# MiraPurkrabek/ProbPose_code

Hardware: AMD Instinct MI355X
Metric: person-crops/sec @ 256x192 bs64 (higher is better)
Workload: dtype f16x3; 1 GPU; ProbPose-small (ViT-S 12x384, 12 heads x 32) bs64 random 256x192 uint8 crops per GPU, flip_test=True, seeded random-init weights: preprocess -> backbone x2 passes -> ProbMapHead (heatmap branch + Sparsemax + 4 towers) -> ProbMap decode -> results in pinned host memory; crops_per_gpu=64, global_batch=64, parallelism=dp1, steps_in_flight=2

## Files before the change

probpose_code_amd/csrc/pp_panel_split.hip:

```cpp
#include "pp_common.h"
#include "pp_device.h"
#include "pp_gemm.h"
#include "pp_split.h"

#include <cstdlib>

namespace pp {
namespace psplit {

#ifndef PSPLIT_DBG
#define PSPLIT_DBG 0
#endif
constexpr int DBG = PSPLIT_DBG;

constexpr int THREADS = 512;
constexpr int CST_BYTES = 48 * 1024;
constexpr int lds_bytes(int BM, int BN, int NST) { return NST * (BM + BN) * 128 + (NST == 2 ? CST_BYTES : 0); }
template <bool SPLIT>
__device__ __forceinline__ f32x4 mma(const u32x4& a, const u32x4& b, f32x4 c) {
    return SPLIT ? mma_f16(a, b, c) : mma_bf16(a, b, c);
}

template <int GATHER, int RF, int CF, bool SPLIT, int NST, bool HEAD = false, bool POOL = false>
__global__ __launch_bounds__(THREADS, 2) void panel_split_kernel(const GemmParams p) {
    constexpr int ESZ = SPLIT ? 4 : 2;
    constexpr int KS = 128 / ESZ;
    constexpr int BM = 32 * RF, BN = 64 * CF;
    constexpr int NA = BM / 8, JA = NA / 8;
    constexpr int STAGE = (BM + BN) * 128;
    constexpr int NI = (BM + BN) / 64;
    constexpr int OFF_CST = NST * STAGE;
    static_assert(NST == 2 || NST == 3, "two or three stages");
    static_assert((BM / 4) * BN * 4 <= (NST == 2 ? CST_BYTES : STAGE), "a quarter of the fp32 tile fits the staging region");
    static_assert(lds_bytes(BM, BN, NST) <= 160 * 1024, "LDS");
    static_assert(NA % 8 == 0 && JA <= 4 && RF % 2 == 0 && (BM + BN) % 64 == 0, "instruction split");
    extern __shared__ __attribute__((aligned(16))) char smem[];
    const int tid = threadIdx.x, lane = tid & 63;
    const int wv = __builtin_amdgcn_readfirstlane(tid >> 6);
    const int rg = wv >> 2, cg = wv & 3;
    const int f_row = lane & 15, f_kg = lane >> 4;

    const int ntn = p.N / BN, ntm = (p.M + BM - 1) / BM;
    const int ntiles = ntn * ntm * p.groups;
    const int nsteps = p.K / KS;
    const int cps = p.Cin / KS;
    const int nprob = p.ksplit > 1 ? p.groups / p.ksplit : p.groups;
    const int cslice = p.ksplit > 1 ? p.Cin / p.ksplit : p.Cin;

    auto decode_tile = [&](int t, int& z, int& m0, int& n0) __attribute__((always_inline)) {
        if ((ntiles & 7) == 0) t = (t & 7) * (ntiles >> 3) + (t >> 3);
        if (p.tile_order == 1) {
            m0 = (t % ntm) * BM;
            const int r = t / ntm;
            n0 = (r % ntn) * BN;
            z = r / ntn;
            return;
        }
        n0 = (t % ntn) * BN;
        const int r = t / ntn;
        z = r % p.groups;
        m0 = (r / p.groups) * BM;
    };

    const int d_l = lane >> 3;
    const unsigned d_kbytes = (unsigned)(((lane & 7) ^ d_l) << 4);
    unsigned a_voff[JA];
    int a_y[JA], a_x[JA];
    unsigned w_voff;
    __amdgpu_buffer_rsrc_t a_rsrc, w_rsrc;
    int i_tile = blockIdx.x, i_step = 0, i_tap = 0, i_c0 = 0, i_py = 0, i_px = 0, i_cbeg = 0;
    bool i_live = true;
    auto setup_issue_tile = [&]() __attribute__((always_inline)) {
        int z = 0, m0 = 0, n0 = 0;
        i_live = i_tile < ntiles;
        if (i_live) decode_tile(i_tile, z, m0, n0);
        i_cbeg = 0;
        if (p.ksplit > 1) {
            i_cbeg = (z / nprob) * cslice;
            z = z % nprob;
        }
        if (GATHER == G_DECONV) {
            i_py = p.py < 0 ? (z >> 1) : p.py;
            i_px = p.py < 0 ? (z & 1) : p.px;
        }
        const char* Act = reinterpret_cast<const char*>(p.A) + (size_t)z * p.strideA_z * ESZ;
        const char* Wt = reinterpret_cast<const char*>(p.W) + (size_t)z * p.strideW_z * ESZ;
        a_rsrc = buffer_rsrc(Act, p.a_bytes);
        w_rsrc = buffer_rsrc(Wt, p.w_bytes);
#pragma unroll
        for (int j = 0; j < JA; ++j) {
            const int m = m0 + 8 * (wv + 8 * j) + d_l;
            const bool ok = i_live && m < p.M;
            if (GATHER == G_LINEAR) {
                a_y[j] = ok ? 0 : -100000;
                a_x[j] = 0;
                a_voff[j] = (unsigned)m * (unsigned)(p.lda * ESZ) + d_kbytes;
            } else {
                const int hw = p.H * p.Wd;
                const int b = m / hw, rr = m - b * hw;
                a_y[j] = ok ? rr / p.Wd : -100000;
                a_x[j] = rr - (rr / p.Wd) * p.Wd;
                a_voff[j] = (unsigned)m * (unsigned)(p.Cin * ESZ) + d_kbytes;
            }
        }
        w_voff = (unsigned)(n0 + 8 * (wv + 8 * JA - NA) + d_l) * (unsigned)(p.ldw * ESZ) + d_kbytes;
        i_step = 0;
        i_tap = 0;
        i_c0 = i_cbeg;
    };
    auto issue_instr = [&](int buf, int j) __attribute__((always_inline)) {
        char* dst = smem + buf * STAGE + (wv + 8 * j) * 1024;
        if (j < JA) {
            int dy = 0, dx = 0;
            if (GATHER == G_CONV3) {
                dy = i_tap / 3 - 1;
                dx = i_tap - (i_tap / 3) * 3 - 1;
            } else if (GATHER == G_DECONV) {
                dy = (i_tap >> 1) - 1 + i_py;
                dx = (i_tap & 1) - 1 + i_px;
            }
            const int jj = j < JA ? j : 0;
            const int yy = a_y[jj] + dy, xx = a_x[jj] + dx;
            const bool ok = GATHER == G_LINEAR ? a_y[jj] >= 0 : (yy >= 0 && yy < p.H && xx >= 0 && xx < p.Wd);
            const int tap_off = GATHER == G_LINEAR ? i_c0 * ESZ : ((dy * p.Wd + dx) * p.Cin + i_c0) * ESZ;
            const unsigned va = ok ? (unsigned)((int)a_voff[jj] + tap_off) : kOob;
            dma16(a_rsrc, dst, va);
        } else {
            const unsigned kb = (unsigned)((i_tap * p.Cin + i_c0) * ESZ) + (unsigned)((j - JA) * 64) * (unsigned)(p.ldw * ESZ);
            dma16(w_rsrc, dst, i_live ? w_voff + kb : kOob);
        }
    };
    const int ntaps = p.K / cslice;
    auto advance_cursor = [&]() __attribute__((always_inline)) {
        const bool ti = p.tap_inner != 0;
        const int tap = i_tap + (ti ? 1 : 0), c0 = i_c0 + (ti ? 0 : KS);
        const bool wrap = ti ? tap == ntaps : c0 == i_cbeg + cslice;
        i_tap = ti ? (wrap ? 0 : tap) : tap + (wrap ? 1 : 0);
        i_c0 = ti ? c0 + (wrap ? KS : 0) : (wrap ? i_cbeg : c0);
        if (++i_step == nsteps) {
            i_tile += gridDim.x;
            setup_issue_tile();
        }
    };
    (void)cps;

    const int sw = f_row & 7;
    const int a_frag_off = (rg * (BM / 2) + f_row) * 128;
    const int w_frag_off = BM * 128 + (cg * (BN / 4) + f_row) * 128;
    auto frag_a = [&](int buf, int lo, int rf) __attribute__((always_inline)) -> u32x4 {
        return *reinterpret_cast<const u32x4*>(smem + buf * STAGE + (((lo * 4 + f_kg) ^ sw) << 4) + a_frag_off + rf * 2048);
    };
    auto frag_w = [&](int buf, int lo, int cf) __attribute__((always_inline)) -> u32x4 {
        return *reinterpret_cast<const u32x4*>(smem + buf * STAGE + (((lo * 4 + f_kg) ^ sw) << 4) + w_frag_off + cf * 2048);
    };

    if ((int)blockIdx.x >= ntiles) return;

    constexpr int HP_PITCH = 100, HP_MAXN = 28;
    constexpr int OFF_HEADB = 4 * HP_MAXN * HP_PITCH * 4;
    static_assert(!HEAD || (SPLIT && GATHER == G_DECONV && RF == 6 && CF == 4 && NST == 2 && OFF_HEADB + 128 <= CST_BYTES), "fused 1x1 head");
    u32x4 hw[HEAD ? 2 : 1][2][2];
    if constexpr (HEAD) {
#pragma unroll
        for (int kb2 = 0; kb2 < 2; ++kb2)
#pragma unroll
            for (int nf = 0; nf < 2; ++nf)
#pragma unroll
                for (int hl = 0; hl < 2; ++hl)
                    hw[kb2][nf][hl] = *reinterpret_cast<const u32x4*>(reinterpret_cast<const char*>(p.head_w) +
                                                                      ((size_t)(((cg * 2 + kb2) * 2 + nf) * 2 + hl) * 64 + lane) * 16);
        if (tid < HP_MAXN) reinterpret_cast<float*>(smem + OFF_CST + OFF_HEADB)[tid] = tid < p.head_n ? p.head_b[tid] : 0.f;
    }
    setup_issue_tile();
#pragma unroll
    for (int s = 0; s < NST; ++s) {
#pragma unroll
        for (int j = 0; j < NI; ++j) issue_instr(s, j);
        advance_cursor();
    }
    wait_vm_lgkm<(NST - 1) * NI>();
    __builtin_amdgcn_s_barrier();
    int cb = 0;
    u32x4 ah[RF], wh[CF], al[RF], wl[CF];
#pragma unroll
    for (int cf = 0; cf < CF; ++cf) wh[cf] = frag_w(0, 0, cf);
#pragma unroll
    for (int rf = 0; rf < RF; ++rf) ah[rf] = frag_a(0, 0, rf);

    for (int tile = blockIdx.x; tile < ntiles; tile += gridDim.x) {
        f32x4 acc[CF][RF];
#pragma unroll
        for (int cf = 0; cf < CF; ++cf)
#pragma unroll
            for (int rf = 0; rf < RF; ++rf) acc[cf][rf] = f32x4{0.f, 0.f, 0.f, 0.f};
        f32x4 bias_r[CF];
        {
            int zb, mb, nb0;
            decode_tile(tile, zb, mb, nb0);
#pragma unroll
            for (int cf = 0; cf < CF; ++cf)
                bias_r[cf] = (p.bias && !(DBG & 1)) ? *reinterpret_cast<const f32x4*>(p.bias + (size_t)zb * p.strideBias_z + nb0 + cg * (BN / 4) + cf * 16 + f_kg * 4)
                                                    : f32x4{0.f, 0.f, 0.f, 0.f};
        }

        for (int k = 0; k < nsteps; ++k) {
            const int nb = cb + 1 == NST ? 0 : cb + 1;
            __builtin_amdgcn_sched_barrier(0);
#pragma unroll
            for (int cf = 0; cf < CF; ++cf) wl[cf] = frag_w(cb, 1, cf);
#pragma unroll
            for (int rf = 0; rf < RF; ++rf) al[rf] = frag_a(cb, 1, rf);
#pragma unroll
            for (int rf = 0; rf < RF; ++rf)
#pragma unroll
                for (int cf = 0; cf < CF; ++cf) acc[cf][rf] = mma<SPLIT>(wh[cf], ah[rf], acc[cf][rf]);
            __builtin_amdgcn_sched_barrier(0);
            wait_vm_lgkm<NST == 2 ? 0 : NI>();
            __builtin_amdgcn_s_barrier();
            __builtin_amdgcn_sched_barrier(0);
            if (NST == 2 || k + 1 < nsteps) {
#pragma unroll
                for (int j = 0; j < NI; ++j) issue_instr(cb, j);
                advance_cursor();
            }
            if constexpr (SPLIT) {
#pragma unroll
                for (int rf = 0; rf < RF; ++rf) {
#pragma unroll
                    for (int cf = 0; cf < CF; ++cf) acc[cf][rf] = mma<SPLIT>(wl[cf], ah[rf], acc[cf][rf]);
                    ah[rf] = frag_a(nb, 0, rf);
                }
#pragma unroll
                for (int cf = 0; cf < CF; ++cf) {
#pragma unroll
                    for (int rf = 0; rf < RF; ++rf) acc[cf][rf] = mma<SPLIT>(wh[cf], al[rf], acc[cf][rf]);
                    wh[cf] = frag_w(nb, 0, cf);
                }
            } else {
#pragma unroll
                for (int cf = 0; cf < CF; ++cf) wh[cf] = frag_w(nb, 0, cf);
#pragma unroll
                for (int rf = 0; rf < RF; ++rf) ah[rf] = frag_a(nb, 0, rf);
#pragma unroll
                for (int rf = 0; rf < RF; ++rf)
#pragma unroll
                    for (int cf = 0; cf < CF; ++cf) acc[cf][rf] = mma<SPLIT>(wl[cf], al[rf], acc[cf][rf]);
            }
            cb = nb;
        }
        const int last_buf = cb == 0 ? NST - 1 : cb - 1;

        if (DBG & 128) {
            f32x4 sum = acc[0][0];
#pragma unroll
            for (int cf = 0; cf < CF; ++cf)
#pragma unroll
                for (int rf = 0; rf < RF; ++rf) sum += acc[cf][rf];
            if (p.M < 0) reinterpret_cast<f32x4*>(p.C)[tid] = sum;
            if (NST == 3) {
#pragma unroll
                for (int j = 0; j < NI; ++j) issue_instr(last_buf, j);
                advance_cursor();
            }
            continue;
        }
        int lane_e = lane;
        asm volatile("" : "+v"(lane_e));
        const int e_row = lane_e & 15, e_kg = lane_e >> 4, tid_e = (tid & ~63) | lane_e;
        int z, m0, n0;
        decode_tile(tile, z, m0, n0);
        if constexpr (HEAD) {
            float* part = reinterpret_cast<float*>(smem + OFF_CST);
            const float* hb = reinterpret_cast<const float*>(smem + OFF_CST + OFF_HEADB);
            const int hwp = p.H * p.Wd;
            const int phase = p.py < 0 ? z : 2 * p.py + p.px;
#pragma unroll
            for (int r = 0; r < 2; ++r) {
                if (rg == r) {
#pragma unroll
                    for (int rf = 0; rf < RF; ++rf) {
                        f32x4 o0 = {0.f, 0.f, 0.f, 0.f}, o1 = {0.f, 0.f, 0.f, 0.f};
#pragma unroll
                        for (int kb2 = 0; kb2 < 2; ++kb2) {
                            f32x4 v0 = acc[2 * kb2][rf] + bias_r[2 * kb2], v1 = acc[2 * kb2 + 1][rf] + bias_r[2 * kb2 + 1];
                            f16x8 ph, pl;
                            {
                                u32x4 phu, plu;
#pragma unroll
                                for (int j = 0; j < 2; ++j) {
                                    unsigned h_, l_;
                                    split_pair(relu_keep_nan(v0[2 * j]), relu_keep_nan(v0[2 * j + 1]), h_, l_);
                                    phu[j] = h_; plu[j] = l_;
                                    split_pair(relu_keep_nan(v1[2 * j]), relu_keep_nan(v1[2 * j + 1]), h_, l_);
                                    phu[2 + j] = h_; plu[2 + j] = l_;
                                }
                                ph = __builtin_bit_cast(f16x8, phu);
                                pl = __builtin_bit_cast(f16x8, plu);
                            }
                            o0 = split_mma(__builtin_bit_cast(f16x8, hw[kb2][0][0]), __builtin_bit_cast(f16x8, hw[kb2][0][1]), ph, pl, o0);
                            o1 = split_mma(__builtin_bit_cast(f16x8, hw[kb2][1][0]), __builtin_bit_cast(f16x8, hw[kb2][1][1]), ph, pl, o1);
                        }
                        const int px = rf * 16 + e_row;
#pragma unroll
                        for (int i = 0; i < 4; ++i) {
                            const int n0_ = 4 * e_kg + i, n1_ = 16 + 4 * e_kg + i;
                            if (n0_ < p.head_n) part[(cg * HP_MAXN + n0_) * HP_PITCH + px] = o0[i];
                            if (n1_ < p.head_n) part[(cg * HP_MAXN + n1_) * HP_PITCH + px] = o1[i];
                        }
                    }
                }
                wait_vm_lgkm<63>();
                __builtin_amdgcn_s_barrier();
                for (int idx = tid_e; idx < p.head_n * 96; idx += THREADS) {
                    const int n = idx / 96, px = idx - n * 96;
                    const int m = m0 + r * 96 + px;
                    if (m >= p.M) continue;
                    const float sum = ((part[(0 * HP_MAXN + n) * HP_PITCH + px] + part[(1 * HP_MAXN + n) * HP_PITCH + px]) +
                                       (part[(2 * HP_MAXN + n) * HP_PITCH + px] + part[(3 * HP_MAXN + n) * HP_PITCH + px])) + hb[n];
                    const int b = m / hwp, rr = m - b * hwp;
                    p.head_out[(((size_t)b * p.head_n + n) * 4 + phase) * hwp + rr] = sum;
                }
                wait_vm_lgkm<63>();
                __builtin_amdgcn_s_barrier();
            }
            continue;
        }
        char* cst = NST == 2 ? smem + OFF_CST : smem + last_buf * STAGE;
        constexpr int ROWB = BN * 4;
        constexpr int LPR = BN / 8;
        constexpr int RPP = THREADS / LPR;
        constexpr int QR = BM / 4;
        constexpr bool RES_PREFETCH = !SPLIT && GATHER == G_LINEAR;
        constexpr int NIT = (QR + RPP - 1) / RPP;
        f32x4 resv[RES_PREFETCH ? NIT : 1][2];
#pragma unroll
        for (int q = 0; q < 4; ++q) {
            if (RES_PREFETCH && p.residual && !(DBG & 2)) {
                const int cl = tid_e % LPR, rl = tid_e / LPR;
#pragma unroll
                for (int it = 0; it < NIT; ++it) {
                    const int ml = it * RPP + rl;
                    const int m = m0 + q * QR + ml;
                    if (rl < RPP && ml < QR && m < p.M) {
                        const float* r = p.residual + (p.res_mod > 0 ? (size_t)(m % p.res_mod) * p.ldres : (size_t)m * p.ldres) + n0 + cl * 8;
                        resv[it][0] = *reinterpret_cast<const f32x4*>(r);
                        resv[it][1] = *reinterpret_cast<const f32x4*>(r + 4);
                    }
                }
            }
            if (rg == (q >> 1)) {
#pragma unroll
                for (int cf = 0; cf < CF; ++cf) {
                    const int nl = cg * (BN / 4) + cf * 16 + e_kg * 4;
                    const f32x4 bv = bias_r[cf];
#pragma unroll
                    for (int r2 = 0; r2 < RF / 2; ++r2) {
                        const int rf = (q & 1) * (RF / 2) + r2;
                        f32x4 v = acc[cf][rf] * p.w_inv + bv;
                        if (p.act == ACT_RELU) {
#pragma unroll
                            for (int j = 0; j < 4; ++j) v[j] = SPLIT ? relu_keep_nan(v[j]) : fmaxf(v[j], 0.f);
                        } else if (p.act == ACT_GELU) {
#pragma unroll
                            for (int j = 0; j < 4; ++j) v[j] = SPLIT ? gelu_erfc_as(v[j]) : gelu_erf(v[j]);
                        }
                        const int ml = r2 * 16 + e_row;
                        *reinterpret_cast<f32x4*>(cst + ml * ROWB + ((((nl >> 2)) ^ (ml & 7)) << 4)) = v;
                    }
                }
            }
            wait_vm_lgkm<63>();
            __builtin_amdgcn_s_barrier();
            const int cl = tid_e % LPR, rl = tid_e / LPR;
            if constexpr (POOL) {
                static_assert(!POOL || (SPLIT && GATHER == G_CONV3 && RF == 6 && NST == 3), "fused pooling: split-fp16 3x3 conv, 192-row tiles");
                const int Wo = p.Wd / p.pool_w;
                if (rl < Wo) {
                    f32x4 v0 = {-3.0e38f, -3.0e38f, -3.0e38f, -3.0e38f}, v1 = v0;
                    for (int r = 0; r < p.pool_h; ++r)
                        for (int c = 0; c < p.pool_w; ++c) {
                            const int ml = r * p.Wd + rl * p.pool_w + c;
                            const f32x4 a0 = *reinterpret_cast<const f32x4*>(cst + ml * ROWB + (((2 * cl) ^ (ml & 7)) << 4));
                            const f32x4 a1 = *reinterpret_cast<const f32x4*>(cst + ml * ROWB + (((2 * cl + 1) ^ (ml & 7)) << 4));
#pragma unroll
                            for (int i = 0; i < 4; ++i) {
                                v0[i] = max_keep_nan(v0[i], a0[i]);
                                v1[i] = max_keep_nan(v1[i], a1[i]);
                            }
                        }
                    f16x8 hv, lv;
#pragma unroll
                    for (int i = 0; i < 4; ++i) {
                        const float b0 = relu_keep_nan(v0[i]), b1 = relu_keep_nan(v1[i]);
                        hv[i] = split_hi(b0);
                        lv[i] = split_lo(b0, hv[i]);
                        hv[4 + i] = split_hi(b1);
                        lv[4 + i] = split_lo(b1, hv[4 + i]);
                    }
                    const int b_img = m0 / (p.H * p.Wd);
                    const size_t eoff = (size_t)z * p.strideC_z + (((size_t)b_img * 4 + q) * Wo + rl) * p.ldc + n0 + cl * 8;
                    if (m0 < p.M) {
                        char* o = split_addr(p.C, eoff);
                        *reinterpret_cast<f16x8*>(o) = hv;
                        *reinterpret_cast<f16x8*>(o + 64) = lv;
                    }
                }
            } else if (rl < RPP) {
#pragma unroll
                for (int it = 0; it < NIT; ++it) {
                    const int ml = it * RPP + rl;
                    const int m = m0 + q * QR + ml;
                    if (ml >= QR || m >= p.M) continue;
                    size_t orow = m;
                    if (GATHER == G_DECONV) {
                        const int hw = p.H * p.Wd;
                        const int b = m / hw, r = m - b * hw;
                        const int y = r / p.Wd, x = r - y * p.Wd;
                        const int py = p.py < 0 ? (z >> 1) : p.py, px = p.py < 0 ? (z & 1) : p.px;
                        orow = ((size_t)b * (2 * p.H) + 2 * y + py) * (2 * p.Wd) + 2 * x + px;
                    }
                    f32x4 v0 = *reinterpret_cast<const f32x4*>(cst + ml * ROWB + (((2 * cl) ^ (ml & 7)) << 4));
                    f32x4 v1 = *reinterpret_cast<const f32x4*>(cst + ml * ROWB + (((2 * cl + 1) ^ (ml & 7)) << 4));
                    const size_t eoff = (size_t)z * p.strideC_z + orow * p.ldc + n0 + cl * 8;
                    if (RES_PREFETCH) {
                        if (p.residual && !(DBG & 2)) {
                            v0 += resv[it][0];
                            v1 += resv[it][1];
                        }
                    } else if (p.residual && !(DBG & 2)) {
                        const float* r = p.residual + (p.res_mod > 0 ? (size_t)(m % p.res_mod) * p.ldres : orow * p.ldres) + n0 + cl * 8;
                        v0 += *reinterpret_cast<const f32x4*>(r);
                        v1 += *reinterpret_cast<const f32x4*>(r + 4);
                    }
                    if (p.out_bf16 == 1) {
                        const bf16x8 ov = {(__bf16)v0[0], (__bf16)v0[1], (__bf16)v0[2], (__bf16)v0[3],
                                           (__bf16)v1[0], (__bf16)v1[1], (__bf16)v1[2], (__bf16)v1[3]};
                        *reinterpret_cast<bf16x8*>(reinterpret_cast<__bf16*>(p.C) + eoff) = ov;
                    } else if (p.out_bf16 == 2) {
                        f16x8 hv, lv;
                        {
                            u32x4 hu, lu;
#pragma unroll
                            for (int j = 0; j < 2; ++j) {
                                unsigned h_, l_;
                                split_pair(v0[2 * j], v0[2 * j + 1], h_, l_);
                                hu[j] = h_; lu[j] = l_;
                                split_pair(v1[2 * j], v1[2 * j + 1], h_, l_);
                                hu[2 + j] = h_; lu[2 + j] = l_;
                            }
                            hv = __builtin_bit_cast(f16x8, hu);
                            lv = __builtin_bit_cast(f16x8, lu);
                        }
                        char* o = split_addr(p.C, eoff);
                        *reinterpret_cast<f16x8*>(o) = hv;
                        *reinterpret_cast<f16x8*>(o + 64) = lv;
                    } else {
                        float* o = reinterpret_cast<float*>(p.C) + eoff;
                        *reinterpret_cast<f32x4*>(o) = v0;
                        *reinterpret_cast<f32x4*>(o + 4) = v1;
                    }
                }
            }
            wait_vm_lgkm<63>();
            __builtin_amdgcn_s_barrier();
        }
        if (NST == 3) wait_vm_lgkm<0>();
        if (NST == 3) {
#pragma unroll
            for (int j = 0; j < NI; ++j) issue_instr(last_buf, j);
            advance_cursor();
        }
    }
}

static int device_cus() {
    static int cus = 0;
    if (cus == 0) {
        int dev = 0;
        hipDeviceProp_t prop;
        if (hipGetDevice(&dev) == hipSuccess && hipGetDeviceProperties(&prop, dev) == hipSuccess) cus = prop.multiProcessorCount;
        if (cus <= 0) cus = 256;
    }
    return cus;
}

}

static int psplit_nst() {
    const int v = option("psplit_nst");
    return v;
}
static int panel_split_shape(const GemmParams& p, int groups) {
    const bool three = psplit_nst() == 3;
    if (p.gather == G_DECONV) return p.N % 256 == 0 ? ((three && !p.head_w) ? 3 : 1) : 0;
    if (p.N % 192 != 0) return 0;
    if (three || p.pool_h > 0) return 4;
    if (p.gather == G_LINEAR && psplit_nst() != 2) {
        const long long cus = 256;
        const long long t2 = (long long)(p.N / 192) * ((p.M + 255) / 256) * groups, t4 = (long long)(p.N / 192) * ((p.M + 191) / 192) * groups;
        const long long c2 = ((t2 + cus - 1) / cus) * 256 * 192, c4 = ((t4 + cus - 1) / cus) * 192 * 192;
        if (c4 * 10 < c2 * 9) return 4;
    }
    return 2;
}

static int panel_linear_min_k(bool out_bf16) {
    const int v = option("panel_linear_mink");
    return v > 0 ? v : (out_bf16 ? 1536 : 768);
}
static bool panel_bf16_conv() {
    const bool v = option("psplit_bf16_conv") != 0;
    return v;
}

static void shape_dims(int shape, int& BM, int& BN) {
    BM = shape == 1 ? 192 : shape == 2 ? 256 : shape == 3 ? 128 : 192;
    BN = shape == 1 ? 256 : shape == 2 ? 192 : shape == 3 ? 256 : 192;
}

bool panel_split_supported(const GemmParams& p, int prec, int groups) {
    if (p.planar_P > 0) return false;
    if (p.ksplit > 1) {
        if (prec != PP_PREC_F16X3 || p.gather != G_CONV3 || p.out_bf16 != 0 || p.bias || p.residual || p.head_w || p.pool_h > 0 || p.act != ACT_NONE) return false;
        if (groups % p.ksplit != 0 || p.Cin % (32 * p.ksplit) != 0 || p.K != 9 * (p.Cin / p.ksplit) || option("psplit_tap_inner") < 1) return false;
    }
    if (p.pool_h > 0) {
        if (prec != PP_PREC_F16X3 || p.gather != G_CONV3 || p.out_bf16 != 2 || p.residual || p.head_w) return false;
        if (p.H * p.Wd != 192 || p.pool_h * p.Wd != 48 || p.H != 4 * p.pool_h || p.Wd % p.pool_w != 0 || p.M % 192 != 0 || p.N % 192 != 0) return false;
        if (p.act != ACT_NONE) return false;
    }
    if (prec == PP_PREC_F16X3) {
        if (p.head_w && !(p.gather == G_DECONV && p.N == 256 && p.head_n >= 1 && p.head_n <= 28)) return false;
        if (p.out_bf16 != 0 && p.out_bf16 != 2) return false;
        if (p.K % 32 != 0 || p.Cin % 32 != 0 || p.ldc % 32 != 0 || p.lda % 32 != 0 || p.ldw % 32 != 0) return false;
        if (p.strideA_z % 32 != 0 || p.strideW_z % 32 != 0 || p.strideC_z % 32 != 0) return false;
    } else if (prec == PP_PREC_BF16) {
        if (p.gather == G_LINEAR ? (p.K < panel_linear_min_k(p.out_bf16 != 0)) : !panel_bf16_conv()) return false;
        if (p.K % 128 != 0 || p.Cin % 64 != 0 || p.head_w) return false;
        if (p.out_bf16 != 0 && p.out_bf16 != 1) return false;
        if (p.ldc % 8 != 0 || p.lda % 8 != 0 || p.ldw % 8 != 0) return false;
    } else {
        return false;
    }
    if (p.residual && (p.out_bf16 == 2 || (p.ldres % 4) != 0)) return false;
    const int shape = panel_split_shape(p, groups);
    if (!shape) return false;
    int BM, BN;
    shape_dims(shape, BM, BN);
    const long long ntiles = (long long)(p.N / BN) * ((p.M + BM - 1) / BM) * groups;
    return ntiles >= 192;
}

int panel_split_gemm(const GemmParams& p_in, int prec, int groups, hipStream_t s) {
    using namespace psplit;
    GemmParams p = p_in;
    p.groups = groups;
    const int ti = option("psplit_tap_inner");
    p.tap_inner = (p.gather == G_CONV3 && ti >= 1) || (p.gather == G_DECONV && ti >= 2) ? 1 : 0;
    PP_REQUIRE(p.ksplit <= 1 || p.tap_inner, PP_ERR_UNSUPPORTED, "pp panel split gemm: split-K slices are channel ranges walked taps-inner");
    p.tile_order = (p.gather == G_CONV3 && p.tap_inner && option("psplit_conv_weight_major") != 0) ? 1 : 0;
    if (p.gather == G_DECONV && option("psplit_deconv_weight_major") != 0) p.tile_order = 1;
    if (p.gather == G_LINEAR) p.Cin = p.K;
    PP_REQUIRE(p.a_bytes > 0 && p.w_bytes > 0 && p.a_bytes < kOob && p.w_bytes < kOob, PP_ERR_UNSUPPORTED,
               "pp panel split gemm: operand tensors must be smaller than 2 GiB (32-bit buffer offsets)");
    void (*kern)(const GemmParams) = nullptr;
    const int shape = panel_split_shape(p, groups);
    int BM, BN;
    shape_dims(shape, BM, BN);
    const bool sp = prec != PP_PREC_BF16;
    if ((long long)p.K * BN * (sp ? 4 : 2) > 3 * 1024 * 1024) p.tile_order = 0;
#define PP_PS(G, RF, CF, NST) (sp ? panel_split_kernel<G, RF, CF, true, NST> : panel_split_kernel<G, RF, CF, false, NST>)
    switch (p.gather) {
        case G_DECONV:
            if (p.head_w) {
                PP_REQUIRE(sp && shape == 1, PP_ERR_UNSUPPORTED, "pp panel split gemm: the fused 1x1 head needs the split-fp16 192 x 256 form");
                kern = panel_split_kernel<G_DECONV, 6, 4, true, 2, true>;
            } else {
                kern = shape == 3 ? PP_PS(G_DECONV, 4, 4, 3) : PP_PS(G_DECONV, 6, 4, 2);
            }
            break;
        case G_CONV3:
            if (p.pool_h > 0) {
                PP_REQUIRE(sp && shape == 4, PP_ERR_UNSUPPORTED, "pp panel split gemm: fused pooling needs the split-fp16 192 x 192 form");
                kern = panel_split_kernel<G_CONV3, 6, 3, true, 3, false, true>;
            } else {
                kern = shape == 4 ? PP_PS(G_CONV3, 6, 3, 3) : PP_PS(G_CONV3, 8, 3, 2);
            }
            break;
        default: kern = shape == 4 ? PP_PS(G_LINEAR, 6, 3, 3) : PP_PS(G_LINEAR, 8, 3, 2); break;
    }
#undef PP_PS
    int slots = device_cus();
    slots -= slots % 8;
    if (p.gather == G_LINEAR && sp && shape == 2 && groups == 1 && p.res_mod == 0 && option("psplit_tail") != 0) {
        const long long ntn = p.N / BN, ntm = (p.M + BM - 1) / BM, tiles = ntn * ntm;
        const long long rounds = tiles / slots, rem = tiles % slots;
        const long long m1 = (rounds * slots / ntn) * BM;
        const long long tail_tiles = m1 < p.M ? ntn * ((p.M - m1 + 127) / 128) : 0;
        if (rounds >= 1 && rem > 0 && rem * 4 <= (long long)slots * 3 && tail_tiles > 0 && tail_tiles <= slots && m1 > 0) {
            GemmParams p1 = p, p2 = p;
            p1.M = (int)m1;
            const size_t a_off = (size_t)m1 * p.lda * 4;
            p2.M = p.M - (int)m1;
            p2.A = reinterpret_cast<const char*>(p.A) + a_off;
            p2.a_bytes = p.a_bytes - (unsigned)a_off;
            p2.C = reinterpret_cast<char*>(p.C) + (size_t)m1 * p.ldc * 4;
            if (p.residual) p2.residual = p.residual + (size_t)m1 * (p.ldres ? p.ldres : p.ldc);
            void (*k1)(const GemmParams) = panel_split_kernel<G_LINEAR, 8, 3, true, 2>;
            void (*k2)(const GemmParams) = panel_split_kernel<G_LINEAR, 4, 3, true, 2>;
            const int lds1 = lds_bytes(256, 192, 2), lds2 = lds_bytes(128, 192, 2);
            PP_HIP_CHECK(hipFuncSetAttribute(reinterpret_cast<const void*>(k1), hipFuncAttributeMaxDynamicSharedMemorySize, lds1));
            PP_HIP_CHECK(hipFuncSetAttribute(reinterpret_cast<const void*>(k2), hipFuncAttributeMaxDynamicSharedMemorySize, lds2));
            hipLaunchKernelGGL(k1, dim3(slots), dim3(THREADS), lds1, s, p1);
            PP_LAUNCH_CHECK();
            hipLaunchKernelGGL(k2, dim3((unsigned)tail_tiles), dim3(THREADS), lds2, s, p2);
            PP_LAUNCH_CHECK();
            return PP_OK;
        }
    }
    const int lds = lds_bytes(BM, BN, shape >= 3 ? 3 : 2);
    const long long ntiles = (long long)(p.N / BN) * ((p.M + BM - 1) / BM) * groups;
    PP_REQUIRE(ntiles < (1ll << 30), PP_ERR_UNSUPPORTED, "pp panel split gemm: too many output tiles");
    const int grid = (int)(ntiles < slots ? ntiles : slots);
    PP_HIP_CHECK(hipFuncSetAttribute(reinterpret_cast<const void*>(kern), hipFuncAttributeMaxDynamicSharedMemorySize, lds));
    hipLaunchKernelGGL(kern, dim3(grid), dim3(THREADS), lds, s, p);
    PP_LAUNCH_CHECK();
    return PP_OK;
}

}
```

Baseline: 14790 crops/s.

## Split deconv GEMM operand staging into separate A and W rings with three-deep weight prefetch

For the split-precision deconv panel kernel (RF=6, CF=4, two stages), the LDS is repartitioned into a 2-deep activation ring and a 3-deep weight ring, each with its own cursor. Weights can then be prefetched a stage further ahead and across tile boundaries, while the epilogue's fp32 staging reuses the idle weight slot plus a smaller 16KB region. The fused 1x1 head epilogue is also restructured to reduce per 16-row fragment with a smaller partial buffer. This adds more cursor bookkeeping and more barrier rounds in the head epilogue, and carries some risk of buffer aliasing bugs between the weight prefetch and the epilogue staging.

```diff
diff --git a/probpose_code_amd/csrc/pp_panel_split.hip b/probpose_code_amd/csrc/pp_panel_split.hip
--- a/probpose_code_amd/csrc/pp_panel_split.hip
+++ b/probpose_code_amd/csrc/pp_panel_split.hip
@@ -21,6 +21,7 @@
     return SPLIT ? mma_f16(a, b, c) : mma_bf16(a, b, c);
 }
 
+constexpr bool OPRING_PLAIN = true;
 template <int GATHER, int RF, int CF, bool SPLIT, int NST, bool HEAD = false, bool POOL = false>
 __global__ __launch_bounds__(THREADS, 2) void panel_split_kernel(const GemmParams p) {
     constexpr int ESZ = SPLIT ? 4 : 2;
@@ -30,6 +31,11 @@
     constexpr int STAGE = (BM + BN) * 128;
     constexpr int NI = (BM + BN) / 64;
     constexpr int OFF_CST = NST * STAGE;
+    constexpr bool OPRING = SPLIT && GATHER == G_DECONV && RF == 6 && CF == 4 && NST == 2 && !POOL && (HEAD || OPRING_PLAIN);
+    constexpr int A_BYTES = BM * 128, W_BYTES = BN * 128, JW = BN / 64;
+    constexpr int OFF_AR = 3 * W_BYTES;
+    constexpr int OFF_EP = OPRING ? OFF_AR + 2 * A_BYTES : OFF_CST, EP_BYTES = OPRING ? 16 * 1024 : CST_BYTES;
+    static_assert(!OPRING || (OFF_EP + EP_BYTES == lds_bytes(BM, BN, NST) && W_BYTES + EP_BYTES == (BM / 4) * BN * 4), "operand rings");
     static_assert(NST == 2 || NST == 3, "two or three stages");
     static_assert((BM / 4) * BN * 4 <= (NST == 2 ? CST_BYTES : STAGE), "a quarter of the fp32 tile fits the staging region");
     static_assert(lds_bytes(BM, BN, NST) <= 160 * 1024, "LDS");
@@ -70,6 +76,8 @@
     __amdgpu_buffer_rsrc_t a_rsrc, w_rsrc;
     int i_tile = blockIdx.x, i_step = 0, i_tap = 0, i_c0 = 0, i_py = 0, i_px = 0, i_cbeg = 0;
     bool i_live = true;
+    int w_tile = blockIdx.x, w_step = 0, w_tap = 0, w_c0 = 0;
+    bool w_live = true;
     auto setup_issue_tile = [&]() __attribute__((always_inline)) {
         int z = 0, m0 = 0, n0 = 0;
         i_live = i_tile < ntiles;
@@ -86,7 +94,7 @@
         const char* Act = reinterpret_cast<const char*>(p.A) + (size_t)z * p.strideA_z * ESZ;
         const char* Wt = reinterpret_cast<const char*>(p.W) + (size_t)z * p.strideW_z * ESZ;
         a_rsrc = buffer_rsrc(Act, p.a_bytes);
-        w_rsrc = buffer_rsrc(Wt, p.w_bytes);
+        if constexpr (!OPRING) w_rsrc = buffer_rsrc(Wt, p.w_bytes);
 #pragma unroll
         for (int j = 0; j < JA; ++j) {
             const int m = m0 + 8 * (wv + 8 * j) + d_l;
@@ -103,13 +111,22 @@
                 a_voff[j] = (unsigned)m * (unsigned)(p.Cin * ESZ) + d_kbytes;
             }
         }
-        w_voff = (unsigned)(n0 + 8 * (wv + 8 * JA - NA) + d_l) * (unsigned)(p.ldw * ESZ) + d_kbytes;
+        if constexpr (!OPRING) w_voff = (unsigned)(n0 + 8 * (wv + 8 * JA - NA) + d_l) * (unsigned)(p.ldw * ESZ) + d_kbytes;
         i_step = 0;
         i_tap = 0;
         i_c0 = i_cbeg;
     };
-    auto issue_instr = [&](int buf, int j) __attribute__((always_inline)) {
-        char* dst = smem + buf * STAGE + (wv + 8 * j) * 1024;
+    auto setup_w_tile = [&]() __attribute__((always_inline)) {
+        int z = 0, m0 = 0, n0 = 0;
+        w_live = w_tile < ntiles;
+        if (w_live) decode_tile(w_tile, z, m0, n0);
+        w_rsrc = buffer_rsrc(reinterpret_cast<const char*>(p.W) + (size_t)z * p.strideW_z * ESZ, p.w_bytes);
+        w_voff = (unsigned)(n0 + 8 * wv + d_l) * (unsigned)(p.ldw * ESZ) + d_kbytes;
+        w_step = 0;
+        w_tap = 0;
+        w_c0 = 0;
+    };
+    auto issue_at = [&](char* dst, int j) __attribute__((always_inline)) {
         if (j < JA) {
             int dy = 0, dx = 0;
             if (GATHER == G_CONV3) {
@@ -126,10 +143,14 @@
             const unsigned va = ok ? (unsigned)((int)a_voff[jj] + tap_off) : kOob;
             dma16(a_rsrc, dst, va);
         } else {
-            const unsigned kb = (unsigned)((i_tap * p.Cin + i_c0) * ESZ) + (unsigned)((j - JA) * 64) * (unsigned)(p.ldw * ESZ);
-            dma16(w_rsrc, dst, i_live ? w_voff + kb : kOob);
-        }
-    };
+            const int tap = OPRING ? w_tap : i_tap, c0 = OPRING ? w_c0 : i_c0;
+            const unsigned kb = (unsigned)((tap * p.Cin + c0) * ESZ) + (unsigned)((j - JA) * 64) * (unsigned)(p.ldw * ESZ);
+            dma16(w_rsrc, dst, (OPRING ? w_live : i_live) ? w_voff + kb : kOob);
+        }
+    };
+    auto issue_instr = [&](int buf, int j) __attribute__((always_inline)) { issue_at(smem + buf * STAGE + (wv + 8 * j) * 1024, j); };
+    auto issue_a = [&](int buf, int j) __attribute__((always_inline)) { issue_at(smem + OFF_AR + buf * A_BYTES + (wv + 8 * j) * 1024, j); };
+    auto issue_w = [&](int buf, int j) __attribute__((always_inline)) { issue_at(smem + buf * W_BYTES + (wv + 8 * j) * 1024, JA + j); };
     const int ntaps = p.K / cslice;
     auto advance_cursor = [&]() __attribute__((always_inline)) {
         const bool ti = p.tap_inner != 0;
@@ -142,23 +163,34 @@
             setup_issue_tile();
         }
     };
+    auto advance_w = [&]() __attribute__((always_inline)) {
+        const bool ti = p.tap_inner != 0;
+        const int tap = w_tap + (ti ? 1 : 0), c0 = w_c0 + (ti ? 0 : KS);
+        const bool wrap = ti ? tap == ntaps : c0 == cslice;
+        w_tap = ti ? (wrap ? 0 : tap) : tap + (wrap ? 1 : 0);
+        w_c0 = ti ? c0 + (wrap ? KS : 0) : (wrap ? 0 : c0);
+        if (++w_step == nsteps) {
+            w_tile += gridDim.x;
+            setup_w_tile();
+        }
+    };
     (void)cps;
 
     const int sw = f_row & 7;
     const int a_frag_off = (rg * (BM / 2) + f_row) * 128;
     const int w_frag_off = BM * 128 + (cg * (BN / 4) + f_row) * 128;
     auto frag_a = [&](int buf, int lo, int rf) __attribute__((always_inline)) -> u32x4 {
-        return *reinterpret_cast<const u32x4*>(smem + buf * STAGE + (((lo * 4 + f_kg) ^ sw) << 4) + a_frag_off + rf * 2048);
+        return *reinterpret_cast<const u32x4*>(smem + (OPRING ? OFF_AR + buf * A_BYTES : buf * STAGE) + (((lo * 4 + f_kg) ^ sw) << 4) + a_frag_off + rf * 2048);
     };
     auto frag_w = [&](int buf, int lo, int cf) __attribute__((always_inline)) -> u32x4 {
-        return *reinterpret_cast<const u32x4*>(smem + buf * STAGE + (((lo * 4 + f_kg) ^ sw) << 4) + w_frag_off + cf * 2048);
+        return *reinterpret_cast<const u32x4*>(smem + (OPRING ? buf * W_BYTES - BM * 128 : buf * STAGE) + (((lo * 4 + f_kg) ^ sw) << 4) + w_frag_off + cf * 2048);
     };
 
     if ((int)blockIdx.x >= ntiles) return;
 
-    constexpr int HP_PITCH = 100, HP_MAXN = 28;
+    constexpr int HP_PITCH = 36, HP_MAXN = 28;
     constexpr int OFF_HEADB = 4 * HP_MAXN * HP_PITCH * 4;
-    static_assert(!HEAD || (SPLIT && GATHER == G_DECONV && RF == 6 && CF == 4 && NST == 2 && OFF_HEADB + 128 <= CST_BYTES), "fused 1x1 head");
+    static_assert(!HEAD || (OPRING && OFF_HEADB + 128 <= EP_BYTES), "fused 1x1 head");
     u32x4 hw[HEAD ? 2 : 1][2][2];
     if constexpr (HEAD) {
 #pragma unroll
@@ -169,18 +201,35 @@
                 for (int hl = 0; hl < 2; ++hl)
                     hw[kb2][nf][hl] = *reinterpret_cast<const u32x4*>(reinterpret_cast<const char*>(p.head_w) +
                                                                       ((size_t)(((cg * 2 + kb2) * 2 + nf) * 2 + hl) * 64 + lane) * 16);
-        if (tid < HP_MAXN) reinterpret_cast<float*>(smem + OFF_CST + OFF_HEADB)[tid] = tid < p.head_n ? p.head_b[tid] : 0.f;
+        if (tid < HP_MAXN) reinterpret_cast<float*>(smem + OFF_EP + OFF_HEADB)[tid] = tid < p.head_n ? p.head_b[tid] : 0.f;
     }
     setup_issue_tile();
-#pragma unroll
-    for (int s = 0; s < NST; ++s) {
-#pragma unroll
-        for (int j = 0; j < NI; ++j) issue_instr(s, j);
-        advance_cursor();
-    }
-    wait_vm_lgkm<(NST - 1) * NI>();
+    if constexpr (OPRING) {
+        setup_w_tile();
+#pragma unroll
+        for (int s = 0; s < 3; ++s) {
+            if (s < 2) {
+#pragma unroll
+                for (int j = 0; j < JA; ++j) issue_a(s, j);
+                advance_cursor();
+            }
+#pragma unroll
+            for (int j = 0; j < JW; ++j) issue_w(s, j);
+            advance_w();
+        }
+        wait_vm_lgkm<JA + 2 * JW>();
+    } else {
+#pragma unroll
+        for (int s = 0; s < NST; ++s) {
+#pragma unroll
+            for (int j = 0; j < NI; ++j) issue_instr(s, j);
+            advance_cursor();
+        }
+        wait_vm_lgkm<(NST - 1) * NI>();
+    }
     __builtin_amdgcn_s_barrier();
     int cb = 0;
+    int cw = 0;
     u32x4 ah[RF], wh[CF], al[RF], wl[CF];
 #pragma unroll
     for (int cf = 0; cf < CF; ++cf) wh[cf] = frag_w(0, 0, cf);
@@ -202,12 +251,19 @@
                 bias_r[cf] = (p.bias && !(DBG & 1)) ? *reinterpret_cast<const f32x4*>(p.bias + (size_t)zb * p.strideBias_z + nb0 + cg * (BN / 4) + cf * 16 + f_kg * 4)
                                                     : f32x4{0.f, 0.f, 0.f, 0.f};
         }
+        if (OPRING && !HEAD && tile != (int)blockIdx.x) {
+            const int last_w = cw == 0 ? 2 : cw - 1;
+#pragma unroll
+            for (int j = 0; j < JW; ++j) issue_w(last_w, j);
+            advance_w();
+        }
 
         for (int k = 0; k < nsteps; ++k) {
             const int nb = cb + 1 == NST ? 0 : cb + 1;
+            const int wb = OPRING ? cw : cb, nwb = OPRING ? (cw == 2 ? 0 : cw + 1) : nb;
             __builtin_amdgcn_sched_barrier(0);
 #pragma unroll
-            for (int cf = 0; cf < CF; ++cf) wl[cf] = frag_w(cb, 1, cf);
+            for (int cf = 0; cf < CF; ++cf) wl[cf] = frag_w(wb, 1, cf);
 #pragma unroll
             for (int rf = 0; rf < RF; ++rf) al[rf] = frag_a(cb, 1, rf);
 #pragma unroll
@@ -215,10 +271,19 @@
 #pragma unroll
                 for (int cf = 0; cf < CF; ++cf) acc[cf][rf] = mma<SPLIT>(wh[cf], ah[rf], acc[cf][rf]);
             __builtin_amdgcn_sched_barrier(0);
-            wait_vm_lgkm<NST == 2 ? 0 : NI>();
+            wait_vm_lgkm<OPRING ? JW : NST == 2 ? 0 : NI>();
             __builtin_amdgcn_s_barrier();
             __builtin_amdgcn_sched_barrier(0);
-            if (NST == 2 || k + 1 < nsteps) {
+            if constexpr (OPRING) {
+#pragma unroll
+                for (int j = 0; j < JA; ++j) issue_a(cb, j);
+                advance_cursor();
+                if (HEAD || k + 1 < nsteps) {
+#pragma unroll
+                    for (int j = 0; j < JW; ++j) issue_w(cw, j);
+                    advance_w();
+                }
+            } else if (NST == 2 || k + 1 < nsteps) {
 #pragma unroll
                 for (int j = 0; j < NI; ++j) issue_instr(cb, j);
                 advance_cursor();
@@ -234,11 +299,11 @@
                 for (int cf = 0; cf < CF; ++cf) {
 #pragma unroll
                     for (int rf = 0; rf < RF; ++rf) acc[cf][rf] = mma<SPLIT>(wh[cf], al[rf], acc[cf][rf]);
-                    wh[cf] = frag_w(nb, 0, cf);
+                    wh[cf] = frag_w(nwb, 0, cf);
                 }
             } else {
 #pragma unroll
-                for (int cf = 0; cf < CF; ++cf) wh[cf] = frag_w(nb, 0, cf);
+                for (int cf = 0; cf < CF; ++cf) wh[cf] = frag_w(nwb, 0, cf);
 #pragma unroll
                 for (int rf = 0; rf < RF; ++rf) ah[rf] = frag_a(nb, 0, rf);
 #pragma unroll
@@ -247,6 +312,7 @@
                     for (int cf = 0; cf < CF; ++cf) acc[cf][rf] = mma<SPLIT>(wl[cf], al[rf], acc[cf][rf]);
             }
             cb = nb;
+            cw = nwb;
         }
         const int last_buf = cb == 0 ? NST - 1 : cb - 1;
 
@@ -270,53 +336,48 @@
         int z, m0, n0;
         decode_tile(tile, z, m0, n0);
         if constexpr (HEAD) {
-            float* part = reinterpret_cast<float*>(smem + OFF_CST);
-            const float* hb = reinterpret_cast<const float*>(smem + OFF_CST + OFF_HEADB);
+            float* part = reinterpret_cast<float*>(smem + OFF_EP);
+            const float* hb = reinterpret_cast<const float*>(smem + OFF_EP + OFF_HEADB);
             const int hwp = p.H * p.Wd;
             const int phase = p.py < 0 ? z : 2 * p.py + p.px;
 #pragma unroll
-            for (int r = 0; r < 2; ++r) {
-                if (rg == r) {
-#pragma unroll
-                    for (int rf = 0; rf < RF; ++rf) {
-                        f32x4 o0 = {0.f, 0.f, 0.f, 0.f}, o1 = {0.f, 0.f, 0.f, 0.f};
-#pragma unroll
-                        for (int kb2 = 0; kb2 < 2; ++kb2) {
-                            f32x4 v0 = acc[2 * kb2][rf] + bias_r[2 * kb2], v1 = acc[2 * kb2 + 1][rf] + bias_r[2 * kb2 + 1];
-                            f16x8 ph, pl;
-                            {
-                                u32x4 phu, plu;
-#pragma unroll
-                                for (int j = 0; j < 2; ++j) {
-                                    unsigned h_, l_;
-                                    split_pair(relu_keep_nan(v0[2 * j]), relu_keep_nan(v0[2 * j + 1]), h_, l_);
-                                    phu[j] = h_; plu[j] = l_;
-                                    split_pair(relu_keep_nan(v1[2 * j]), relu_keep_nan(v1[2 * j + 1]), h_, l_);
-                                    phu[2 + j] = h_; plu[2 + j] = l_;
-                                }
-                                ph = __builtin_bit_cast(f16x8, phu);
-                                pl = __builtin_bit_cast(f16x8, plu);
-                            }
-                            o0 = split_mma(__builtin_bit_cast(f16x8, hw[kb2][0][0]), __builtin_bit_cast(f16x8, hw[kb2][0][1]), ph, pl, o0);
-                            o1 = split_mma(__builtin_bit_cast(f16x8, hw[kb2][1][0]), __builtin_bit_cast(f16x8, hw[kb2][1][1]), ph, pl, o1);
+            for (int rf = 0; rf < RF; ++rf) {
+                f32x4 o0 = {0.f, 0.f, 0.f, 0.f}, o1 = {0.f, 0.f, 0.f, 0.f};
+#pragma unroll
+                for (int kb2 = 0; kb2 < 2; ++kb2) {
+                    f32x4 v0 = acc[2 * kb2][rf] + bias_r[2 * kb2], v1 = acc[2 * kb2 + 1][rf] + bias_r[2 * kb2 + 1];
+                    f16x8 ph, pl;
+                    {
+                        u32x4 phu, plu;
+#pragma unroll
+                        for (int j = 0; j < 2; ++j) {
+                            unsigned h_, l_;
+                            split_pair(relu_keep_nan(v0[2 * j]), relu_keep_nan(v0[2 * j + 1]), h_, l_);
+                            phu[j] = h_; plu[j] = l_;
+                            split_pair(relu_keep_nan(v1[2 * j]), relu_keep_nan(v1[2 * j + 1]), h_, l_);
+                            phu[2 + j] = h_; plu[2 + j] = l_;
                         }
-                        const int px = rf * 16 + e_row;
-#pragma unroll
-                        for (int i = 0; i < 4; ++i) {
-                            const int n0_ = 4 * e_kg + i, n1_ = 16 + 4 * e_kg + i;
-                            if (n0_ < p.head_n) part[(cg * HP_MAXN + n0_) * HP_PITCH + px] = o0[i];
-                            if (n1_ < p.head_n) part[(cg * HP_MAXN + n1_) * HP_PITCH + px] = o1[i];
-                        }
-                    }
+                        ph = __builtin_bit_cast(f16x8, phu);
+                        pl = __builtin_bit_cast(f16x8, plu);
+                    }
+                    o0 = split_mma(__builtin_bit_cast(f16x8, hw[kb2][0][0]), __builtin_bit_cast(f16x8, hw[kb2][0][1]), ph, pl, o0);
+                    o1 = split_mma(__builtin_bit_cast(f16x8, hw[kb2][1][0]), __builtin_bit_cast(f16x8, hw[kb2][1][1]), ph, pl, o1);
+                }
+                const int px = rg * 16 + e_row;
+#pragma unroll
+                for (int i = 0; i < 4; ++i) {
+                    const int n0_ = 4 * e_kg + i, n1_ = 16 + 4 * e_kg + i;
+                    if (n0_ < p.head_n) part[(cg * HP_MAXN + n0_) * HP_PITCH + px] = o0[i];
+                    if (n1_ < p.head_n) part[(cg * HP_MAXN + n1_) * HP_PITCH + px] = o1[i];
                 }
                 wait_vm_lgkm<63>();
                 __builtin_amdgcn_s_barrier();
-                for (int idx = tid_e; idx < p.head_n * 96; idx += THREADS) {
-                    const int n = idx / 96, px = idx - n * 96;
-                    const int m = m0 + r * 96 + px;
+                for (int idx = tid_e; idx < p.head_n * 32; idx += THREADS) {
+                    const int n = idx >> 5, px2 = idx & 31;
+                    const int m = m0 + (px2 >> 4) * (BM / 2) + rf * 16 + (px2 & 15);
                     if (m >= p.M) continue;
-                    const float sum = ((part[(0 * HP_MAXN + n) * HP_PITCH + px] + part[(1 * HP_MAXN + n) * HP_PITCH + px]) +
-                                       (part[(2 * HP_MAXN + n) * HP_PITCH + px] + part[(3 * HP_MAXN + n) * HP_PITCH + px])) + hb[n];
+                    const float sum = ((part[(0 * HP_MAXN + n) * HP_PITCH + px2] + part[(1 * HP_MAXN + n) * HP_PITCH + px2]) +
+                                       (part[(2 * HP_MAXN + n) * HP_PITCH + px2] + part[(3 * HP_MAXN + n) * HP_PITCH + px2])) + hb[n];
                     const int b = m / hwp, rr = m - b * hwp;
                     p.head_out[(((size_t)b * p.head_n + n) * 4 + phase) * hwp + rr] = sum;
                 }
@@ -327,6 +388,11 @@
         }
         char* cst = NST == 2 ? smem + OFF_CST : smem + last_buf * STAGE;
         constexpr int ROWB = BN * 4;
+        const int last_w = cw == 0 ? 2 : cw - 1;
+        auto cst_row = [&](int ml) __attribute__((always_inline)) -> char* {
+            if constexpr (OPRING) return smem + ml * ROWB + (ml < W_BYTES / ROWB ? last_w * W_BYTES : OFF_EP - W_BYTES);
+            else return cst + ml * ROWB;
+        };
         constexpr int LPR = BN / 8;
         constexpr int RPP = THREADS / LPR;
         constexpr int QR = BM / 4;
@@ -365,7 +431,7 @@
                             for (int j = 0; j < 4; ++j) v[j] = SPLIT ? gelu_erfc_as(v[j]) : gelu_erf(v[j]);
                         }
                         const int ml = r2 * 16 + e_row;
-                        *reinterpret_cast<f32x4*>(cst + ml * ROWB + ((((nl >> 2)) ^ (ml & 7)) << 4)) = v;
+                        *reinterpret_cast<f32x4*>(cst_row(ml) + ((((nl >> 2)) ^ (ml & 7)) << 4)) = v;
                     }
                 }
             }
@@ -380,8 +446,8 @@
                     for (int r = 0; r < p.pool_h; ++r)
                         for (int c = 0; c < p.pool_w; ++c) {
                             const int ml = r * p.Wd + rl * p.pool_w + c;
-                            const f32x4 a0 = *reinterpret_cast<const f32x4*>(cst + ml * ROWB + (((2 * cl) ^ (ml & 7)) << 4));
-                            const f32x4 a1 = *reinterpret_cast<const f32x4*>(cst + ml * ROWB + (((2 * cl + 1) ^ (ml & 7)) << 4));
+                            const f32x4 a0 = *reinterpret_cast<const f32x4*>(cst_row(ml) + (((2 * cl) ^ (ml & 7)) << 4));
+                            const f32x4 a1 = *reinterpret_cast<const f32x4*>(cst_row(ml) + (((2 * cl + 1) ^ (ml & 7)) << 4));
 #pragma unroll
                             for (int i = 0; i < 4; ++i) {
                                 v0[i] = max_keep_nan(v0[i], a0[i]);
@@ -419,8 +485,8 @@
                         const int py = p.py < 0 ? (z >> 1) : p.py, px = p.py < 0 ? (z & 1) : p.px;
                         orow = ((size_t)b * (2 * p.H) + 2 * y + py) * (2 * p.Wd) + 2 * x + px;
                     }
-                    f32x4 v0 = *reinterpret_cast<const f32x4*>(cst + ml * ROWB + (((2 * cl) ^ (ml & 7)) << 4));
-                    f32x4 v1 = *reinterpret_cast<const f32x4*>(cst + ml * ROWB + (((2 * cl + 1) ^ (ml & 7)) << 4));
+                    f32x4 v0 = *reinterpret_cast<const f32x4*>(cst_row(ml) + (((2 * cl) ^ (ml & 7)) << 4));
+                    f32x4 v1 = *reinterpret_cast<const f32x4*>(cst_row(ml) + (((2 * cl + 1) ^ (ml & 7)) << 4));
                     const size_t eoff = (size_t)z * p.strideC_z + orow * p.ldc + n0 + cl * 8;
                     if (RES_PREFETCH) {
                         if (p.residual && !(DBG & 2)) {
```

Result: no change. 14790 crops/s, median of 2 (-0.0%).
